# AberHu/TF-NAS

Measured on AMD Instinct MI355X. Metric: supernet search images/sec (w-step + alpha-step), higher is better.
Workload: dtype fp32

## Files before the change

### tf-nas_amd/csrc/gemm_kernels.hip

```cpp
#include <stdlib.h>
#include <string.h>
#include "gemm_core.h"
#include "gemm_x3.h"
#include "kernels.h"
#include "prof.h"

__device__ __forceinline__ f32x4 stem_patch4(const float* __restrict__ img, const TfnasCellDesc& d, int p, int t0) {
    const int HW = d.H * d.W, n = p / HW, r = p - n * HW, ho = r / d.W, wo = r - ho * d.W;
    f32x4 v = zero4();
#pragma unroll
    for (int j = 0; j < 4; ++j) {
        const int t = t0 + j;
        if (t < 27) {
            const int ci = t / 9, rem = t - 9 * ci, ky = rem / 3, kx = rem - 3 * ky;
            const int hi = 2 * ho + ky - 1, wi = 2 * wo + kx - 1;
            if (hi >= 0 && hi < d.Hi && wi >= 0 && wi < d.Wi) v[j] = img[((size_t)(n * 3 + ci) * d.Hi + hi) * d.Wi + wi];
        }
    }
    return v;
}

constexpr int kLbBig = 3, kLbSmall = 4;
constexpr int kLbX3Big = 2, kLbX3Small = 3;
constexpr int gemm_lb(int nt, int mm) { return mm == 0 ? (nt >= 5 ? kLbBig : kLbSmall) : (nt >= 5 ? kLbX3Big : kLbX3Small); }
// ... 460 lines not shown
    const int ocp = (oc + 15) & ~15;
    const int r0 = blockIdx.x * rows_per_split, r1 = min(Po, r0 + rows_per_split);
    const int nchunks = (r1 - r0 + 15) >> 4;
    const int tid = threadIdx.x, lane = tid & 63, lr = lane & 15, lq = lane >> 4, wrow = (tid >> 6) * 32;

    const Bn3Tab tab = bn3_tab_fill(lds + T::LDS_FLOATS, ocp, d, g, stats3, red3, wmix);
    const int mch = m0 + (tid & 31) * 4;
    const bool chok = mch < mcp;
    const size_t acol = (size_t)off + min(mch, mcp - 4);
    float2 c2[4];
#pragma unroll
    for (int j = 0; j < 4; ++j)
        c2[j] = (mch + j < mc) ? bn_consts(stats2 + 2 * (size_t)(off + mch + j), 1.0 / (double)Po, d.eps)
                               : make_float2(0.f, 0.f);
    __syncthreads();
    constexpr int BQ = T::BN / 4;
    int bcol[T::B_ITERS];
    bool bok[T::B_ITERS];
    f32x4 k_mean[T::B_ITERS], k_a3[T::B_ITERS], k_ab[T::B_ITERS], k_s[T::B_ITERS];
#pragma unroll
    for (int i = 0; i < T::B_ITERS; ++i) {
        const int idx = tid + 256 * i, o = n0 + (idx % BQ) * 4;
        bok[i] = idx < T::B_ITEMS && o < oc;
        bcol[i] = min(o, oc - 4);
#pragma unroll
        for (int j = 0; j < 4; ++j) {
            const int oo = bcol[i] + j;
            k_mean[i][j] = tab.mean[oo];
            k_a3[i][j] = tab.a3[oo];
            k_ab[i][j] = tab.a3[oo] * tab.b3[oo];
            k_s[i][j] = tab.rstd[oo] * tab.c3[oo] * tab.a3[oo];
        }
    }
    const float inv_hw = 1.f / (float)HW;
    const bool small_p = Po < (1 << 24);
    auto image_of = [&](int p) -> int {
        if (!small_p) return p / HW;
        int q = (int)((float)p * inv_hw);
        const int r = p - q * HW;
        q += (r >= HW) ? 1 : 0;
        q -= (r < 0) ? 1 : 0;
        return q;
    };

    f32x4 acc[2][NT];
    acc_zero<NT>(acc);
    auto la = [&](int c, int i, int kl, int m) -> Raw2 {
        const int p = min(r0 + c * 16 + kl, r1 - 1);
        Raw2 r;
        r.a = ld4(D + ((size_t)p * M + acol));
        r.b = ld4(gbase + ((size_t)image_of(p) * M + acol) * se01);
        return r;
    };
    auto xa = [&](Raw2 r, int c, int i, int kl, int m) -> f32x4 {
        f32x4 v = r.a;
#pragma unroll
        for (int j = 0; j < 4; ++j) v[j] = act_f<ACT>((v[j] - c2[j].x) * c2[j].y);
        if (has_se) v *= r.b;
        return (chok && r0 + c * 16 + kl < r1) ? v : zero4();
    };
    auto lb = [&](int c, int i, int kl, int n) -> Raw2 {
        const int p = min(r0 + c * 16 + kl, r1 - 1);
        Raw2 r;
        r.a = ld4(dout + (size_t)p * oc + bcol[i]);
        r.b = ld4(Pr + ((size_t)g * Po + p) * oc + bcol[i]);
        return r;
    };
    auto xb = [&](Raw2 r, int c, int i, int kl, int n) -> f32x4 {
        const f32x4 v = (k_a3[i] * r.a - k_ab[i]) - (r.b - k_mean[i]) * k_s[i];
        return (bok[i] && r0 + c * 16 + kl < r1) ? v : zero4();
    };
    gemm_mainloop2<NT, false, false, false>(la, xa, lb, xb, nchunks, acc, lds);
    const bool vec = (mc & 3) == 0;
#pragma unroll
    for (int i = 0; i < 2; ++i) {
        const int ch0 = m0 + wrow + 16 * i + 4 * lq;
#pragma unroll
        for (int j = 0; j < NT; ++j) {
            const int o = n0 + 16 * j + lr;
            if (o >= oc) continue;
            float* dst = gw + (size_t)o * mc + ch0;
            if (vec && ch0 + 3 < mc) {
                st4(dst, acc[i][j]);
            } else {
#pragma unroll
                for (int r = 0; r < 4; ++r)
                    if (ch0 + r < mc) dst[r] = acc[i][j][r];
            }
        }
    }
}

__device__ __forceinline__ f32x4 bn1_de(const f32x4* cb, f32x4 deh, f32x4 e) {
    f32x4 r;
#pragma unroll
    for (int j = 0; j < 4; ++j) {
        const f32x4 t = cb[j];
        const float eh = (e[j] - t.x) * t.y;
        r[j] = t.y * (deh[j] - t.z - eh * t.w);
    }
    return r;
}

__device__ __forceinline__ f32x4 sink_add(f32x4 v, float w, f32x4 g) {
    float px = w * g.x, py = w * g.y, pz = w * g.z, pw = w * g.w;
    asm volatile("" : "+v"(px), "+v"(py), "+v"(pz), "+v"(pw));
    f32x4 r;
    r.x = v.x + px; r.y = v.y + py; r.z = v.z + pz; r.w = v.w + pw;
    return r;
}

template <int NT, int MM>
__global__ __launch_bounds__(256, gemm_lb(NT, MM)) void k_expand_dgrad(TfnasCellDesc d, const float* __restrict__ dEh,
                                                      const float* __restrict__ x, const float* __restrict__ cb1,
                                                      const float* __restrict__ gram, const float* __restrict__ dout,
                                                      const float* __restrict__ wmix, float* __restrict__ dx,
                                                      float* __restrict__ dxp, int nsplit,
                                                      const float* __restrict__ add_src,
                                                      const float* __restrict__ add_scale, int xonly_slot = -1) {
    using T = GT<NT>;
    __shared__ __attribute__((aligned(16))) float lds[T::LDS_FLOATS];
    const int n0 = blockIdx.y * T::BN;
    const int P = d.N * d.H * d.W, ic = d.ic, M = d.M;
    const int nrt = (P + 127) >> 7;
    const int tid = threadIdx.x, lr = tid & 15, wrow = (tid >> 6) * 32;
    const int zs = (int)blockIdx.z;
    int mchunks = 0;
    for (int g = 0; g < d.G; ++g) mchunks += (d.g[g].mcp + 15) >> 4;
    const int nchunks_all = mchunks + ((ic + 15) >> 4);
    const bool xonly = xonly_slot >= 0;
    const int per = xonly ? nchunks_all - mchunks : (nchunks_all + nsplit - 1) / nsplit;
    const int cbeg = xonly ? mchunks : zs * per;
    const int nchunks = max(0, min(nchunks_all, cbeg + per) - cbeg);
    float* __restrict__ dst = xonly ? dxp + (size_t)xonly_slot * P * ic : (nsplit > 1 ? dxp + (size_t)blockIdx.z * P * ic : dx);
    const bool plain = nsplit == 1 && !xonly;
    const bool add_res = d.has_res && plain;
    const bool add_sink = add_src != nullptr && plain;
    const float sink_w = add_src ? add_scale[0] : 0.f;
    float sumw = 1.f;
    if (wmix) {
        sumw = 0.f;
        for (int g = 0; g < d.G; ++g) sumw += wmix[g];
    }

    for (int rt = blockIdx.x; rt < nrt; rt += gridDim.x) {
        f32x4 acc[2][NT];
        acc_zero<NT>(acc);
        bool is_x;
        int k0, klim_a, klim_b, ld_a;
        size_t aoff;
        const float* bsrc;
        const float* ssrc;
        auto pre = [&](int c) {
            c += cbeg;
            if (c >= mchunks) {
                is_x = true;
                k0 = (c - mchunks) * 16;
                klim_a = klim_b = ld_a = ic;
                aoff = 0;
                bsrc = gram;
                ssrc = cb1 + 1;
                return;
            }
            int g = 0;
            for (; g < d.G - 1; ++g) {
                const int t = (d.g[g].mcp + 15) >> 4;
                if (c < t) break;
                c -= t;
            }
            is_x = false;
            k0 = c * 16;
            klim_a = d.g[g].mcp;
            klim_b = d.g[g].mc;
            ld_a = M;
            aoff = d.g[g].off;
            bsrc = d.g[g].w_expand;
            ssrc = cb1 + 4 * (size_t)d.g[g].off + 1;
        };
        int prow[2];
#pragma unroll
        for (int i = 0; i < 2; ++i) prow[i] = rt * 128 + wrow + 16 * i + lr;
        auto la = [&](int c, int i, int kl) -> f32x4 {
            const int pc = min(prow[i], P - 1), k = min(k0 + kl, klim_a - 4);
            return ld4((is_x ? x : dEh) + (size_t)pc * ld_a + aoff + k);
        };
        auto xa = [&](f32x4 r, int c, int i, int kl) -> f32x4 {
            return (prow[i] < P && k0 + kl < klim_a) ? r : zero4();
        };
        auto lb = [&](int c, int kl, int n) -> RawWS {
            const int kc = min(k0 + kl, klim_b - 1), col = min(n0 + n, ic - 4);
            RawWS r;
            r.w = ld4(bsrc + (size_t)kc * ic + col);
            r.s = ssrc[is_x ? 0 : 4 * (size_t)kc];
            return r;
        };
        auto xb = [&](RawWS r, int c, int kl, int n) -> f32x4 {
            const f32x4 v = is_x ? -r.w : splat4(r.s) * r.w;
            return (n0 + n < ic && k0 + kl < klim_b) ? v : zero4();
        };
        gemm_adirect<NT, false, MM>(pre, la, xa, lb, xb, nchunks, acc, lds);
        emit_tile_rows<NT>(acc, lds, [&](int lrow, int lc, f32x4 v) {
            const int p = rt * 128 + lrow, c = n0 + lc;
            if (p < P && c < ic) {
                if (plain) v += ld4(gram + (size_t)ic * ic + c);
                if (add_res) v += splat4(sumw) * ld4(dout + (size_t)p * d.oc + c);
                if (add_sink) v = sink_add(v, sink_w, ld4(add_src + (size_t)p * ic + c));
                st4(dst + (size_t)p * ic + c, v);
            }
        });
    }
}

__global__ __launch_bounds__(256) void k_dx_reduce(TfnasCellDesc d, const float* __restrict__ dxp, int nsplit,
                                                   const float* __restrict__ gram, const float* __restrict__ dout,
                                                   const float* __restrict__ wmix, float* __restrict__ dx,
                                                   const float* __restrict__ add_src,
                                                   const float* __restrict__ add_scale) {
    const float sink_w = add_src ? add_scale[0] : 0.f;
    const size_t n4 = (size_t)d.N * d.H * d.W * d.ic / 4;
    const int iq = d.ic / 4;
    const float* __restrict__ bias = gram + (size_t)d.ic * d.ic;
    float sumw = 1.f;
    if (wmix) {
        sumw = 0.f;
        for (int g = 0; g < d.G; ++g) sumw += wmix[g];
    }
    for (size_t i = (size_t)blockIdx.x * 256 + threadIdx.x; i < n4; i += (size_t)gridDim.x * 256) {
        f32x4 v = ld4(bias + 4 * (int)(i % iq));
        if (d.has_res) v += splat4(sumw) * ld4(dout + 4 * i);
        for (int z = 0; z < nsplit; ++z) v += ld4(dxp + (size_t)z * n4 * 4 + 4 * i);
        if (add_src) v = sink_add(v, sink_w, ld4(add_src + 4 * i));
        st4(dx + 4 * i, v);
    }
}

template <int NT>
__global__ __launch_bounds__(256) void k_expand_gram(TfnasCellDesc d, const float* __restrict__ cb1, int chunks_per_split,
                                                     int nsplit, float* __restrict__ part) {
    using T = GT<NT>;
    __shared__ __attribute__((aligned(16))) float lds[T::LDS_FLOATS];
    const int ic = d.ic;
    const int m0 = blockIdx.y * 128, n0 = blockIdx.z * T::BN;
    const int xs = (int)blockIdx.x;
    int mchunks = 0;
    for (int g = 0; g < d.G; ++g) mchunks += (d.g[g].mcp + 15) >> 4;
    const int cbeg = xs * chunks_per_split;
    const int nchunks = max(0, min(mchunks, cbeg + chunks_per_split) - cbeg);
    const f32x4* cb = reinterpret_cast<const f32x4*>(cb1);
    const int tid = threadIdx.x, lane = tid & 63, lr = lane & 15, lq = lane >> 4, wrow = (tid >> 6) * 32;
    float* __restrict__ out = part + (size_t)blockIdx.x * (size_t)(ic + 4) * ic;

    f32x4 acc[2][NT];
    acc_zero<NT>(acc);
    auto locate = [&](int c, int& g, int& k0) {
        c += cbeg;
        g = 0;
        for (; g < d.G - 1; ++g) {
            const int t = (d.g[g].mcp + 15) >> 4;
            if (c < t) break;
            c -= t;
        }
        k0 = c * 16;
    };
    auto fa = [&](int c, int kl, int m) -> f32x4 {
        int g, k0;
        locate(c, g, k0);
        const int k = k0 + kl, r = m0 + m;
        if (k >= d.g[g].mc || r > ic) return zero4();
        const f32x4 t = cb[d.g[g].off + k];
        const float sk = t.y * t.y * t.w;
        if (r == ic) {
            f32x4 v = zero4();
            v.x = sk * t.x - t.y * t.z;
            return v;
        }
        return splat4(sk) * ld4(d.g[g].w_expand + (size_t)k * ic + r);
    };
    auto fb = [&](int c, int kl, int n) -> f32x4 {
        int g, k0;
        locate(c, g, k0);
        const int k = k0 + kl;
        return (k < d.g[g].mc && n0 + n < ic) ? ld4(d.g[g].w_expand + (size_t)k * ic + n0 + n) : zero4();
    };
    gemm_mainloop<NT, false, false>(fa, fb, nchunks, acc, lds);
#pragma unroll
    for (int i = 0; i < 2; ++i)
#pragma unroll
        for (int r = 0; r < 4; ++r) {
            const int row = m0 + wrow + 16 * i + 4 * lq + r;
            if (row <= ic) {
#pragma unroll
                for (int j = 0; j < NT; ++j) {
                    const int cc = n0 + 16 * j + lr;
                    if (cc < ic) out[(size_t)row * ic + cc] = acc[i][j][r];
                }
            }
        }
}

#ifndef GRAM1_MAX_K
#define GRAM1_MAX_K 1536
#endif
constexpr int GRAM1_GB = 8;
template <int GRAM1_NW>
__global__ __launch_bounds__(64 * GRAM1_NW) void k_gram1(TfnasCellDesc d, const float* __restrict__ cb1, float* __restrict__ gram) {
    __shared__ float part[GRAM1_NW][2][16][17];
    const int ic = d.ic;
    const int r0 = blockIdx.y * 16, c0 = blockIdx.x * 32;
    const int tid = threadIdx.x, wave = tid >> 6, lane = tid & 63, li = lane & 15, kq = lane >> 4;
    const f32x4* cb = reinterpret_cast<const f32x4*>(cb1);
    const int r = r0 + li, ca = c0 + li, cb_ = c0 + 16 + li;
    const bool row_w = r < ic, row_b = r == ic, oka = ca < ic, okb = cb_ < ic;
    const int ra = row_w ? r : 0, caa = oka ? ca : 0, cbb = okb ? cb_ : 0;
    f32x4 acc0 = zero4(), acc1 = zero4();
    int base = 0;
    for (int g = 0; g < d.G; ++g) {
        const float* __restrict__ W = d.g[g].w_expand;
        const int mc = d.g[g].mc, off = d.g[g].off;
        const int nstep = (mc + 3) >> 2, nbatch = (nstep + GRAM1_GB - 1) / GRAM1_GB;
        int b = (wave - base % GRAM1_NW + GRAM1_NW) % GRAM1_NW;
        for (; b < nbatch; b += GRAM1_NW) {
            const int s0 = b * GRAM1_GB;
            float a[GRAM1_GB], b0[GRAM1_GB], b1[GRAM1_GB];
            f32x4 t[GRAM1_GB];
#pragma unroll
            for (int u = 0; u < GRAM1_GB; ++u) {
                const int m = 4 * (s0 + u) + kq;
                const int mm = m < mc ? m : mc - 1;
                const float* wr = W + (size_t)mm * ic;
                t[u] = cb[off + mm];
                a[u] = wr[ra];
                b0[u] = wr[caa];
                b1[u] = wr[cbb];
            }
#pragma unroll
            for (int u = 0; u < GRAM1_GB; ++u) {
                const int m = 4 * (s0 + u) + kq;
                const bool okm = m < mc;
                const float sk = t[u].y * t[u].y * t[u].w;
                float av = row_w ? sk * a[u] : (row_b ? sk * t[u].x - t[u].y * t[u].z : 0.f);
                av = okm ? av : 0.f;
                const float bv0 = (okm && oka) ? b0[u] : 0.f, bv1 = (okm && okb) ? b1[u] : 0.f;
                acc0 = __builtin_amdgcn_mfma_f32_16x16x4f32(av, bv0, acc0, 0, 0, 0);
                acc1 = __builtin_amdgcn_mfma_f32_16x16x4f32(av, bv1, acc1, 0, 0, 0);
            }
        }
        base += nbatch;
    }
#pragma unroll
    for (int q = 0; q < 4; ++q) {
        part[wave][0][4 * kq + q][li] = acc0[q];
        part[wave][1][4 * kq + q][li] = acc1[q];
    }
    __syncthreads();
    for (int e = tid; e < 512; e += 64 * GRAM1_NW) {
        const int h = e >> 8, row = (e >> 4) & 15, col = e & 15;
        double v = 0.0;
#pragma unroll
        for (int w = 0; w < GRAM1_NW; ++w) v += (double)part[w][h][row][col];
        const int rr = r0 + row, cc = c0 + 16 * h + col;
        if (rr <= ic && cc < ic) gram[(size_t)rr * ic + cc] = (float)v;
    }
}

template <int NT, bool STEM, bool XG>
__global__ __launch_bounds__(256, wgrad_lb(NT)) void k_expand_wgrad(TfnasCellDesc d, const float* __restrict__ dEh,
                                                      const float* __restrict__ E, const float* __restrict__ cb1,
                                                      const float* __restrict__ x, int rows_per_split,
                                                      float* __restrict__ part, size_t out_size, size_t out_main) {
    using T = GT<NT>;
    __shared__ __attribute__((aligned(16))) float lds[T::LDS_FLOATS];
    const int ic = d.ic;
    int ty = blockIdx.y, g = 0;
    for (; g < d.G - 1; ++g) {
        const int t = (d.g[g].mcp + 127) >> 7;
        if (ty < t) break;
        ty -= t;
    }
    const int mc = d.g[g].mc, mcp = d.g[g].mcp, off = d.g[g].off;
    const bool last = XG && g == d.G - 1;
    size_t poff = 0;
    for (int gg = 0; gg < g; ++gg) poff += (size_t)d.g[gg].mc * ic;
    float* __restrict__ gw = part + (size_t)blockIdx.x * out_size + poff;
    float* __restrict__ gx = part + (size_t)blockIdx.x * out_size + out_main;
    const int m0 = ty * 128, n0 = blockIdx.z * T::BN;
    const int P = d.N * d.H * d.W, M = d.M;
    const int r0 = blockIdx.x * rows_per_split, r1 = min(P, r0 + rows_per_split);
    const int nchunks = (r1 - r0 + 15) >> 4;
    const int tid = threadIdx.x, lane = tid & 63, lr = lane & 15, lq = lane >> 4, wrow = (tid >> 6) * 32;

    const int mch = m0 + (tid & 31) * 4;
    const bool chok = mch < mcp;
    const size_t acol = (size_t)off + min(mch, mcp - 4);
    f32x4 k_mu = zero4(), k_r = zero4(), k_rt1 = zero4(), k_s = zero4();
    if (!XG) {
#pragma unroll
        for (int j = 0; j < 4; ++j) {
            const f32x4 t = (mch + j < mcp) ? reinterpret_cast<const f32x4*>(cb1)[off + mch + j] : zero4();
            k_mu[j] = t.x;
            k_r[j] = t.y;
            k_rt1[j] = t.y * t.z;
            k_s[j] = t.y * t.y * t.w;
        }
    }
    const int ext = mch - mcp;
    const bool ax = last && ext >= 0 && ext < ic, aone = last && ext == ic;
    const float* __restrict__ abase = ax ? x + ext : dEh + acol;
    const size_t apitch = ax ? (size_t)ic : (size_t)M;
    const bool aok = chok || ax;
    constexpr int BQ = T::BN / 4;
    int bcol[T::B_ITERS];
    bool bok[T::B_ITERS];
#pragma unroll
    for (int i = 0; i < T::B_ITERS; ++i) {
        const int idx = tid + 256 * i, cc = n0 + (idx % BQ) * 4;
        bok[i] = idx < T::B_ITEMS && cc < ic;
        bcol[i] = STEM ? cc : min(cc, ic - 4);
    }

    f32x4 acc[2][NT];
    acc_zero<NT>(acc);
    auto la = [&](int c, int i, int kl, int m) -> Raw2 {
        const int p = min(r0 + c * 16 + kl, r1 - 1);
        Raw2 r;
        if (XG) {
            r.a = ld4(abase + (size_t)p * apitch);
            r.b = r.a;
        } else {
            const size_t at = (size_t)p * M + acol;
            r.a = ld4(dEh + at);
            r.b = ld4(E + at);
        }
        return r;
    };
    auto xa = [&](Raw2 r, int c, int i, int kl, int m) -> f32x4 {
        if (XG) {
            f32x4 v = aok ? r.a : zero4();
            if (aone) v.x = 1.f;
            return (r0 + c * 16 + kl < r1) ? v : zero4();
        }
        const f32x4 v = (k_r * r.a - k_rt1) - (r.b - k_mu) * k_s;
        return (chok && r0 + c * 16 + kl < r1) ? v : zero4();
    };
    auto lb = [&](int c, int i, int kl, int n) -> f32x4 {
        if (STEM) {
            const int p = r0 + c * 16 + kl;
            return (p < r1 && bok[i]) ? stem_patch4(x, d, p, bcol[i]) : zero4();
        }
        const int p = min(r0 + c * 16 + kl, r1 - 1);
        return ld4(x + (size_t)p * ic + bcol[i]);
    };
    auto xb = [&](f32x4 r, int c, int i, int kl, int n) -> f32x4 {
        if (STEM) return r;
        return (bok[i] && r0 + c * 16 + kl < r1) ? r : zero4();
    };
    gemm_mainloop2<NT, false, false, false>(la, xa, lb, xb, nchunks, acc, lds);
#pragma unroll
    for (int i = 0; i < 2; ++i)
#pragma unroll
        for (int r = 0; r < 4; ++r) {
            const int ch = m0 + wrow + 16 * i + 4 * lq + r;
            float* __restrict__ row = nullptr;
            if (ch < mc) row = gw + (size_t)ch * ic;
            else if (last && ch >= mcp && ch - mcp <= ic) row = gx + (size_t)(ch - mcp) * ic;
            if (row) {
#pragma unroll
                for (int j = 0; j < NT; ++j) {
                    const int cc = n0 + 16 * j + lr;
                    if (cc < ic) row[cc] = acc[i][j][r];
                }
            }
        }
}

__global__ __launch_bounds__(256) void k_expand_wgrad_fix(TfnasCellDesc d, const float* __restrict__ cb1,
                                                          const double* __restrict__ red, size_t out_main) {
    __shared__ double ps[4][64];
    const int ic = d.ic, lane = threadIdx.x & 63, wv = threadIdx.x >> 6;
    const size_t e = (size_t)blockIdx.x * 64 + lane;
    const bool ok = e < out_main;
    int g = 0;
    size_t poff = 0;
    for (; g < d.G - 1; ++g) {
        const size_t n = (size_t)d.g[g].mc * ic;
        if (e < poff + n) break;
        poff += n;
    }
    const int m = ok ? (int)((e - poff) / ic) : 0, c = ok ? (int)(e - poff - (size_t)m * ic) : 0;
    const double* __restrict__ Gx = red + out_main;
    const float* __restrict__ w = d.g[g].w_expand + (size_t)m * ic;
    double wg0 = 0.0, wg1 = 0.0;
    for (int k = 4 * wv; k < ic; k += 16) {
        const f32x4 wq = ld4(w + k);
        wg0 += (double)wq.x * Gx[(size_t)k * ic + c] + (double)wq.z * Gx[(size_t)(k + 2) * ic + c];
        wg1 += (double)wq.y * Gx[(size_t)(k + 1) * ic + c] + (double)wq.w * Gx[(size_t)(k + 3) * ic + c];
    }
    ps[wv][lane] = wg0 + wg1;
    __syncthreads();
    if (wv == 0 && ok) {
        const double wg = (ps[0][lane] + ps[1][lane]) + (ps[2][lane] + ps[3][lane]);
        const f32x4 t = reinterpret_cast<const f32x4*>(cb1)[d.g[g].off + m];
        const double sx = Gx[(size_t)ic * ic + c], mu = t.x, r = t.y, t1 = t.z, t2 = t.w;
        const float v = (float)(r * (red[e] - t1 * sx - t2 * r * (wg - mu * sx)));
        float* __restrict__ o = d.g[g].g_expand + (e - poff);
        *o = (d.flags & TFNAS_CELL_ACCUM_WGRAD) ? *o + v : v;
    }
}

static const int kNtSmall[] = {1, 2, 3, 4, 5, 7};
static constexpr int kGtLdsFloats[8] = {0, GT<1>::LDS_FLOATS, GT<2>::LDS_FLOATS, GT<3>::LDS_FLOATS, GT<4>::LDS_FLOATS,
                                        GT<5>::LDS_FLOATS, 0, GT<7>::LDS_FLOATS};

#define NT_CASE(n, ...) case n: { constexpr int NT = n; __VA_ARGS__; } break;
#define DISPATCH_NT_GROUPS(nt, ...)   \
    switch (nt) {                     \
        NT_CASE(4, __VA_ARGS__)       \
        NT_CASE(5, __VA_ARGS__)       \
        NT_CASE(7, __VA_ARGS__)       \
        default: return TFNAS_EINVAL; \
    }
#define DISPATCH_NT(nt, ...)                         \
    switch (nt) {                                    \
        NT_CASE(1, __VA_ARGS__)                      \
        NT_CASE(2, __VA_ARGS__)                      \
        NT_CASE(3, __VA_ARGS__)                      \
        default: DISPATCH_NT_GROUPS(nt, __VA_ARGS__) \
    }
#define DISPATCH_MM(mode, ...)                                 \
    switch (mode) {                                            \
        case 0: { constexpr int MM = 0; __VA_ARGS__; } break;  \
        case 1: { constexpr int MM = 1; __VA_ARGS__; } break;  \
        case 3: { constexpr int MM = 3; __VA_ARGS__; } break;  \
        default: { constexpr int MM = 6; __VA_ARGS__; } break; \
    }
#define DISPATCH_ACT(act, ...) ACT_DISPATCH(act, __VA_ARGS__)

static int g_gemm_mode = 6;
int gemm_mode() { return g_gemm_mode & 7; }
int set_gemm_mode(int m) {
    const int base = m & ~TFNAS_GEMM_EVERYWHERE;
    if (base != 0 && base != 1 && base != 3 && base != 6) return TFNAS_EINVAL;
    g_gemm_mode = m;
    return 0;
}
static inline int gemm_word(const TfnasCellDesc& d) { return (d.gemm_mode & TFNAS_GEMM_EXPLICIT) ? d.gemm_mode : g_gemm_mode; }
int gemm_mode_of(const TfnasCellDesc& d) { return gemm_word(d) & 7; }
static int gemm_arith(const TfnasCellDesc& d, bool dgrad) {
    for (int g = 0; g < d.G; ++g)
        if (d.g[g].mc & 3) return 0;
    const int m = gemm_mode_of(d);
    if (!dgrad || m == 0 || (gemm_word(d) & TFNAS_GEMM_EVERYWHERE)) return m;
    if (m == 1) return m;
    return (d.G > 1 && d.Ho * d.Wo <= 196) ? m : 0;
}
static inline int gemm_slots(int nt, int mm) { return 256 * gemm_lb(nt, mm); }

static size_t stats_row_cap(size_t row_floats) {
    const size_t fit = TFNAS_PART_FLOATS / (row_floats ? row_floats : 1);
    return fit < 1024 ? fit : 1024;
}

static int row_blocks(int rows, int other_blocks, size_t cap, int slots, int max_gx = 1024) {
    const int nrt = cdiv(rows, 128);
    const int other = other_blocks > 0 ? other_blocks : 1;
    int lim = nrt;
    if ((size_t)lim > cap) lim = (int)cap;
    if (lim > max_gx) lim = max_gx;
    if (lim < 1) lim = 1;
    long best_cost = -1;
    int best = 1;
    for (int gx = 1; gx <= lim; ++gx) {
        const long cost = (long)cdiv(gx * other, slots) * cdiv(nrt, gx);
        if (best_cost < 0 || cost <= best_cost) {
            best_cost = cost;
            best = gx;
        }
    }
    return best;
}

static int pick_nt_groups(const TfnasCellDesc& d) {
    int min_mcp = 1 << 30;
    for (int g = 0; g < d.G; ++g) min_mcp = d.g[g].mcp < min_mcp ? d.g[g].mcp : min_mcp;
    if (min_mcp >= 200) return 4;
    static const int cands[] = {4, 5, 7};
    int best = 4;
    long best_pad = -1;
    for (int i = 0; i < 3; ++i) {
        long pad = 0;
        for (int g = 0; g < d.G; ++g) pad += (long)cdiv(d.g[g].mcp, 16 * cands[i]) * 16 * cands[i];
        if (best_pad < 0 || pad < best_pad || (pad == best_pad && cands[i] > best)) {
            best_pad = pad;
            best = cands[i];
        }
    }
    return best;
}
static int group_tiles(const TfnasCellDesc& d, int width, int last_extra = 0) {
    int t = 0;
    for (int g = 0; g < d.G; ++g) t += cdiv(d.g[g].mcp + (g == d.G - 1 ? last_extra : 0), width);
    return t;
}
static int max_mcp(const TfnasCellDesc& d) {
    int m = 0;
    for (int g = 0; g < d.G; ++g) m = d.g[g].mcp > m ? d.g[g].mcp : m;
    return m;
}
static size_t mid_floats(const TfnasCellDesc& d, int n) {
    size_t f = 0;
    for (int g = 0; g < d.G; ++g) f += (size_t)d.g[g].mc * n;
    return f;
}
static GemmPlan plan_cols(int n) {
    GemmPlan p{};
    p.nt = pick_nt(n, kNtSmall, 6);
    p.tiles = cdiv(n, 16 * p.nt);
    return p;
}

GemmPlan gemm_plan_expand_fwd(const TfnasCellDesc& d) {
    GemmPlan p{};
    p.var = d.mode == TFNAS_MODE_STEM ? GEMM_STEM : GEMM_PLAIN;
    p.nt = p.var == GEMM_STEM ? (d.g[0].mcp <= 32 ? 2 : 4) : pick_nt_groups(d);
    p.mm = gemm_arith(d, false);
    p.tiles = group_tiles(d, 16 * p.nt);
    p.grid = dim3(row_blocks(d.N * d.H * d.W, p.tiles, stats_row_cap(2 * (size_t)d.M), gemm_slots(p.nt, p.mm)), p.tiles);
    return p;
}

int launch_expand_fwd(const TfnasCellDesc& d, const float* x, float* E, double* stats1, float* part,
                      hipStream_t s) {
    ProfScope _prof(TK_EXPAND_FWD, s);
    const GemmPlan p = gemm_plan_expand_fwd(d);
    DISPATCH_MM(p.mm, {
        if (p.var == GEMM_STEM)
            hipLaunchKernelGGL((p.nt == 2 ? k_expand_fwd<2, true, MM> : k_expand_fwd<4, true, MM>), p.grid, dim3(256), 0, s, d, x, E, part);
        else
            DISPATCH_NT_GROUPS(p.nt, { hipLaunchKernelGGL((k_expand_fwd<NT, false, MM>), p.grid, dim3(256), 0, s, d, x, E, part); })
    })
    _prof.stop();
    return launch_reduce_rows(part, p.grid.x, 2 * d.M, 2 * (size_t)d.M, stats1, nullptr, s);
}

#ifndef TFNAS_WSPLIT_DGRAD
#define TFNAS_WSPLIT_DGRAD 2
#endif
#ifndef TFNAS_WSPLIT_PFWD
#define TFNAS_WSPLIT_PFWD 2
#endif
GemmPlan gemm_plan_project_fwd(const TfnasCellDesc& d) {
    GemmPlan p = plan_cols(d.oc);
    p.mm = gemm_arith(d, false);
    const int mcp_max = max_mcp(d), ncols2 = 2 * d.G * d.oc;
    const int Po = d.N * d.Ho * d.Wo, nrt = cdiv(Po, 128);
    p.shm = (kGtLdsFloats[p.nt] + 2 * ((mcp_max + 15) & ~15)) * sizeof(float);
    int nsplit = 1;
    const int wgs = nrt * p.tiles * d.G, kch = cdiv(mcp_max, 16);
    if (wgs < 512 && kch >= 16 && (d.oc & 3) == 0 && d.oc <= 1024) {
        nsplit = cdiv(1024, wgs);
        if (nsplit > 4) nsplit = 4;
        if (nsplit > kch / 8) nsplit = kch / 8;
        if (d.need_wgrad && d.G == 1 && nsplit > TFNAS_WSPLIT_PFWD) nsplit = TFNAS_WSPLIT_PFWD;
        const size_t per = (size_t)d.G * Po * d.oc, rows2 = 256 * (size_t)ncols2;
        while (nsplit > 1 && (nsplit - 1) * per + rows2 > TFNAS_PART_FLOATS) --nsplit;
    }
    p.splits = nsplit;
    p.parts = nsplit - 1;
    if (p.parts) p.grid = dim3(nrt, p.tiles, d.G * nsplit);
    else p.grid = dim3(row_blocks(Po, p.tiles * d.G, stats_row_cap((size_t)ncols2), gemm_slots(p.nt, p.mm)), p.tiles, d.G);
    int gx2 = cdiv(Po, 64);
    if (gx2 > 256) gx2 = 256;
    p.rps = cdiv(Po, gx2);
    p.grid2 = dim3(cdiv(Po, p.rps), d.G);
    return p;
}

int launch_project_fwd(const TfnasCellDesc& d, const float* D, const float* gate, const double* stats2,
                       float* Pr, double* stats3, float* part, hipStream_t s) {
    ProfScope _prof(TK_PROJECT_FWD, s);
    const GemmPlan p = gemm_plan_project_fwd(d);
    const int ncols2 = 2 * d.G * d.oc, Po = d.N * d.Ho * d.Wo;
    float* prp = p.parts ? part : nullptr;
    float* rows = part + (size_t)p.parts * d.G * Po * d.oc;
    DISPATCH_MM(p.mm, DISPATCH_NT(p.nt, DISPATCH_ACT(d.act, {
        hipLaunchKernelGGL((k_project_fwd<NT, ACT, MM>), p.grid, dim3(256), p.shm, s, d, D, gate, stats2, Pr, part, p.splits, prp);
    })))
    if (p.parts) hipLaunchKernelGGL(k_pr_reduce, p.grid2, dim3(256), 0, s, Pr, prp, p.parts, d.G, Po, d.oc, p.rps, rows);
    _prof.stop();
    return launch_reduce_rows(rows, p.parts ? p.grid2.x : p.grid.x, ncols2, (size_t)ncols2, stats3, nullptr, s);
}

GemmPlan gemm_plan_project_dgrad(const TfnasCellDesc& d, bool fold) {
    GemmPlan p{};
    p.var = fold ? GEMM_FOLD : GEMM_PLAIN;
    p.nt = pick_nt_groups(d);
    p.mm = gemm_arith(d, true);
    p.tiles = group_tiles(d, 16 * p.nt);
    p.grid = dim3(row_blocks(d.N * d.Ho * d.Wo, p.tiles, 1u << 30, gemm_slots(p.nt, p.mm)), p.tiles);
    p.shm = (kGtLdsFloats[p.nt] + 4 * ((d.oc + 15) & ~15)) * sizeof(float);
    return p;
}

int launch_project_dgrad(const TfnasCellDesc& d, const float* dout, const float* Pr, const double* stats3,
                         const double* red3, const float* wmix, float* dZ, hipStream_t s, const float* D,
                         const double* stats2, float* rec) {
    ProfScope _prof(TK_PROJECT_DGRAD, s);
    if (rec && (!D || !stats2)) return TFNAS_ENULL;
    if (rec && d.act != TFNAS_ACT_RELU && d.act != TFNAS_ACT_SWISH) return TFNAS_EINVAL;
    const GemmPlan p = gemm_plan_project_dgrad(d, rec != nullptr);
    DISPATCH_MM(p.mm, DISPATCH_NT_GROUPS(p.nt, {
        if (p.var == GEMM_FOLD)
            hipLaunchKernelGGL((k_project_dgrad<NT, MM, true>), p.grid, dim3(256), p.shm, s, d, dout, Pr, stats3, red3, wmix, dZ,
                               D, stats2, rec);
        else
            hipLaunchKernelGGL((k_project_dgrad<NT, MM>), p.grid, dim3(256), p.shm, s, d, dout, Pr, stats3, red3, wmix, dZ);
    }))
    return (int)hipGetLastError();
}

static void plan_row_splits(GemmPlan& p, int rows, int mtiles, int ztiles, size_t scratch) {
    const int target = 256 * wgrad_lb(p.nt), min_rows = 128, out_tiles = mtiles * ztiles;
    int splits = target / (out_tiles > 0 ? out_tiles : 1);
    const size_t cap = scratch / (p.out > 0 ? p.out : 1);
    if ((size_t)splits > cap) splits = (int)cap;
    if (splits < 1) splits = 1;
    int rps = cdiv(rows, splits);
    if (rps < min_rows) rps = min_rows;
    p.rps = ((rps + 15) / 16) * 16;
    p.splits = cdiv(rows, p.rps);
    p.grid = dim3(p.splits, mtiles, ztiles);
}
static int reduce_group_wgrads(const TfnasCellDesc& d, const GemmPlan& p, const float* part, int n, float* TfnasGroup::*dst,
                               hipStream_t s) {
    size_t poff = 0;
    for (int g = 0; g < d.G; ++g) {
        const int cols = d.g[g].mc * n;
        int rc = launch_reduce_rows(part + poff, p.splits, cols, p.out, nullptr, d.g[g].*dst, s, wgrad_accum(d));
        if (rc) return rc;
        poff += cols;
    }
    return (int)hipGetLastError();
}

GemmPlan gemm_plan_project_wgrad(const TfnasCellDesc& d) {
    GemmPlan p = plan_cols(d.oc);
    p.out = mid_floats(d, d.oc);
    plan_row_splits(p, d.N * d.Ho * d.Wo, cdiv(max_mcp(d), 128), p.tiles * d.G, TFNAS_PART_FLOATS);
    p.shm = (kGtLdsFloats[p.nt] + 5 * ((d.oc + 15) & ~15)) * sizeof(float);
    return p;
}

int launch_project_wgrad(const TfnasCellDesc& d, const float* dout, const float* Pr, const float* D,
                         const float* gate, const double* stats2, const double* stats3, const double* red3,
                         const float* wmix, float* part, hipStream_t s) {
    ProfScope _prof(TK_PROJECT_WGRAD, s);
    const GemmPlan p = gemm_plan_project_wgrad(d);
    DISPATCH_NT(p.nt, DISPATCH_ACT(d.act, {
        hipLaunchKernelGGL((k_project_wgrad<NT, ACT>), p.grid, dim3(256), p.shm, s, d, dout, Pr, D, gate, stats2,
                           stats3, red3, wmix, p.rps, p.tiles, part, p.out);
    }))
    _prof.stop();
    return reduce_group_wgrads(d, p, part, d.oc, &TfnasGroup::g_proj, s);
}

size_t expand_gram_floats(const TfnasCellDesc& d) { return (size_t)(d.ic + 4) * d.ic; }
static int mid_chunks(const TfnasCellDesc& d) { return group_tiles(d, 16); }

GemmPlan gemm_plan_expand_gram(const TfnasCellDesc& d, size_t scratch_floats) {
    GemmPlan p{};
    if (!(d.route & TFNAS_ROUTE_GRAM2) && mid_floats(d, 1) <= GRAM1_MAX_K) {
        p.var = GEMM_GRAM1;
        p.grid = dim3(cdiv(d.ic, 32), cdiv(d.ic + 1, 16));
        return p;
    }
    p = plan_cols(d.ic);
    const size_t gsz = expand_gram_floats(d);
    const int mchunks = mid_chunks(d), mtiles = cdiv(d.ic + 1, 128);
    int splits = cdiv(512, mtiles * p.tiles);
    if (splits > mchunks / 4) splits = mchunks / 4;
    if ((size_t)splits > scratch_floats / gsz) splits = (int)(scratch_floats / gsz);
    if (splits < 1) splits = 1;
    p.rps = cdiv(mchunks, splits);
    p.splits = cdiv(mchunks, p.rps);
    p.grid = dim3(p.splits, mtiles, p.tiles);
    return p;
}

int launch_expand_gram(const TfnasCellDesc& d, const float* cb1, float* scratch, size_t scratch_floats, float* gram,
                       hipStream_t s) {
    ProfScope _prof(TK_SMALL, s);
    const GemmPlan p = gemm_plan_expand_gram(d, scratch_floats);
    if (p.var == GEMM_GRAM1) {
        for (int g = 0; g < d.G; ++g)
            if (d.g[g].mc < 1) return TFNAS_EINVAL;
        if (d.mode == TFNAS_MODE_HEAD) hipLaunchKernelGGL(k_gram1<16>, p.grid, dim3(1024), 0, s, d, cb1, gram);
        else hipLaunchKernelGGL(k_gram1<4>, p.grid, dim3(256), 0, s, d, cb1, gram);
        return (int)hipGetLastError();
    }
    const size_t gsz = expand_gram_floats(d);
    if (scratch_floats < gsz) return TFNAS_ERANGE;
    DISPATCH_NT(p.nt, { hipLaunchKernelGGL(k_expand_gram<NT>, p.grid, dim3(256), 0, s, d, cb1, p.rps, p.splits, scratch); })
    _prof.stop();
    return launch_reduce_rows(scratch, p.splits, (int)gsz, gsz, nullptr, gram, s);
}

GemmPlan gemm_plan_expand_dgrad(const TfnasCellDesc& d, bool split, int nsl) {
    GemmPlan p = plan_cols(d.ic);
    p.mm = gemm_arith(d, true);
    const int P = d.N * d.H * d.W, out_tiles = cdiv(P, 128) * p.tiles;
    p.splits = 1;
    if (split && nsl < 0 && out_tiles < 512) {
        const int mchunks = mid_chunks(d);
        int ns = cdiv(1024, out_tiles);
        if (ns > 16) ns = 16;
        if (ns > mchunks / 4) ns = mchunks / 4;
        if (d.need_wgrad && d.G == 1 && ns > TFNAS_WSPLIT_DGRAD) ns = TFNAS_WSPLIT_DGRAD;
        p.splits = ns < 1 ? 1 : ns;
    }
    p.grid = dim3(row_blocks(P, p.tiles * p.splits, 1u << 30, gemm_slots(p.nt, p.mm), 4096), p.tiles, p.splits);
    p.parts = nsl >= 0 ? nsl + 1 : (p.splits > 1 ? p.splits : 0);
    size_t blocks = cdiv64((size_t)P * d.ic / 4, 256 * 2);
    p.grid2 = dim3((unsigned)(blocks > 2048 ? 2048 : blocks));
    return p;
}

int launch_expand_dgrad(const TfnasCellDesc& d, const float* dEh, const float* x, const float* cb1, const float* gram,
                        const float* dout, const float* wmix, float* dx, float* dxp, hipStream_t s,
                        const float* add_src, const float* add_scale, int nsl) {
    const GemmPlan p = gemm_plan_expand_dgrad(d, dxp != nullptr, nsl);
    {
        ProfScope _prof(TK_EXPAND_DGRAD, s);
        DISPATCH_MM(p.mm, DISPATCH_NT(p.nt, {
            hipLaunchKernelGGL((k_expand_dgrad<NT, MM>), p.grid, dim3(256), 0, s, d, dEh, x, cb1, gram, dout, wmix, dx, dxp, p.splits,
                               add_src, add_scale, nsl);
        }))
    }
    if (p.parts) {
        ProfScope _p2(TK_SMALL, s);
        hipLaunchKernelGGL(k_dx_reduce, p.grid2, dim3(256), 0, s, d, dxp, p.parts, gram, dout, wmix, dx, add_src, add_scale);
    }
    return (int)hipGetLastError();
}

static size_t xg_red_floats(const GemmPlan& p) { return p.var == GEMM_XG ? 2 * p.out + 4 : 0; }

GemmPlan gemm_plan_expand_wgrad(const TfnasCellDesc& d) {
    GemmPlan p = plan_cols(d.ic);
    const int P = d.N * d.H * d.W;
    if (d.mode == TFNAS_MODE_STEM) p.var = GEMM_STEM;
    else if (!(d.route & TFNAS_ROUTE_XG_OFF) && (d.ic & 3) == 0 &&
             ((d.route & TFNAS_ROUTE_XG_ALL) || (size_t)P * d.M * sizeof(float) >= ((size_t)100 << 20)))
        p.var = GEMM_XG;
    const int next = p.var == GEMM_XG ? d.ic + 1 : 0;
    p.out_main = mid_floats(d, d.ic);
    p.out = p.out_main + (size_t)next * d.ic;
    plan_row_splits(p, P, group_tiles(d, 128, next), p.tiles, TFNAS_PART_FLOATS - xg_red_floats(p));
    return p;
}

int launch_expand_wgrad(const TfnasCellDesc& d, const float* dEh, const float* E, const float* cb1,
                        const float* x, float* part, hipStream_t s) {
    ProfScope _prof(TK_EXPAND_WGRAD, s);
    const GemmPlan p = gemm_plan_expand_wgrad(d);
    const size_t red_floats = xg_red_floats(p);
    if (p.var != GEMM_XG && !E) return TFNAS_ENULL;
    if (red_floats + p.out > TFNAS_PART_FLOATS) return TFNAS_ERANGE;
    if (p.var == GEMM_STEM && p.nt != 2) return TFNAS_EINVAL;
    DISPATCH_NT(p.nt, {
        auto k = p.var == GEMM_XG ? k_expand_wgrad<NT, false, true> : k_expand_wgrad<NT, false, false>;
        if (p.var == GEMM_STEM) k = k_expand_wgrad<2, true, false>;
        hipLaunchKernelGGL(k, p.grid, dim3(256), 0, s, d, dEh, E, cb1, x, p.rps, part, p.out, p.out_main);
    })
    _prof.stop();
    if (p.var != GEMM_XG) return reduce_group_wgrads(d, p, part, d.ic, &TfnasGroup::g_expand, s);
    double* red = reinterpret_cast<double*>((uintptr_t)(part + TFNAS_PART_FLOATS - red_floats + 3) & ~(uintptr_t)15);
    int rc = launch_reduce_rows(part, p.splits, (int)p.out, p.out, red, nullptr, s);
    if (rc) return rc;
    ProfScope _p2(TK_EXPAND_WGRAD, s);
    hipLaunchKernelGGL(k_expand_wgrad_fix, dim3((unsigned)cdiv64(p.out_main, 64)), dim3(256), 0, s, d, cb1, red, p.out_main);
    return (int)hipGetLastError();
}
```

Before: 3969.

## Parameterize gram1 column tile width and flatten group/batch wave scheduling

The gram1 kernel gets a template column-tile count NT. Non-head cells now use 16-column tiles instead of 32, which doubles the grid along x for more parallelism. Head mode keeps 32 columns. The nested per-group loop with modular wave offsets is replaced by a flat batch index walked across groups, balancing waves over the global batch list. The wave index is made uniform with readfirstlane. A few products are pinned in registers to control codegen, at the cost of more A-operand reloads across column tiles.

```diff
diff --git a/tf-nas_amd/csrc/gemm_kernels.hip b/tf-nas_amd/csrc/gemm_kernels.hip
--- a/tf-nas_amd/csrc/gemm_kernels.hip
+++ b/tf-nas_amd/csrc/gemm_kernels.hip
@@ -786,64 +786,77 @@
 #define GRAM1_MAX_K 1536
 #endif
 constexpr int GRAM1_GB = 8;
-template <int GRAM1_NW>
+template <int GRAM1_NW, int NT>
 __global__ __launch_bounds__(64 * GRAM1_NW) void k_gram1(TfnasCellDesc d, const float* __restrict__ cb1, float* __restrict__ gram) {
-    __shared__ float part[GRAM1_NW][2][16][17];
-    const int ic = d.ic;
-    const int r0 = blockIdx.y * 16, c0 = blockIdx.x * 32;
-    const int tid = threadIdx.x, wave = tid >> 6, lane = tid & 63, li = lane & 15, kq = lane >> 4;
+    __shared__ float part[GRAM1_NW][NT][16][17];
+    const int ic = d.ic, G = d.G;
+    const int r0 = blockIdx.y * 16, c0 = blockIdx.x * 16 * NT;
+    const int tid = threadIdx.x, lane = tid & 63, li = lane & 15, kq = lane >> 4;
+    const int wave = __builtin_amdgcn_readfirstlane(tid >> 6);
     const f32x4* cb = reinterpret_cast<const f32x4*>(cb1);
-    const int r = r0 + li, ca = c0 + li, cb_ = c0 + 16 + li;
-    const bool row_w = r < ic, row_b = r == ic, oka = ca < ic, okb = cb_ < ic;
-    const int ra = row_w ? r : 0, caa = oka ? ca : 0, cbb = okb ? cb_ : 0;
-    f32x4 acc0 = zero4(), acc1 = zero4();
-    int base = 0;
-    for (int g = 0; g < d.G; ++g) {
+    const int r = r0 + li;
+    const bool row_w = r < ic, row_b = r == ic;
+    const int ra = row_w ? r : 0;
+    bool okc[NT];
+    int cc[NT];
+    f32x4 acc[NT];
+#pragma unroll
+    for (int j = 0; j < NT; ++j) {
+        const int c = c0 + 16 * j + li;
+        okc[j] = c < ic;
+        cc[j] = okc[j] ? c : 0;
+        acc[j] = zero4();
+    }
+    int g = 0, b = wave;
+    for (;; b += GRAM1_NW) {
+        int mc = 0;
+        for (; g < G; ++g) {
+            mc = d.g[g].mc;
+            const int nbatch = (((mc + 3) >> 2) + GRAM1_GB - 1) / GRAM1_GB;
+            if (b < nbatch) break;
+            b -= nbatch;
+        }
+        if (g == G) break;
         const float* __restrict__ W = d.g[g].w_expand;
-        const int mc = d.g[g].mc, off = d.g[g].off;
-        const int nstep = (mc + 3) >> 2, nbatch = (nstep + GRAM1_GB - 1) / GRAM1_GB;
-        int b = (wave - base % GRAM1_NW + GRAM1_NW) % GRAM1_NW;
-        for (; b < nbatch; b += GRAM1_NW) {
-            const int s0 = b * GRAM1_GB;
-            float a[GRAM1_GB], b0[GRAM1_GB], b1[GRAM1_GB];
-            f32x4 t[GRAM1_GB];
-#pragma unroll
-            for (int u = 0; u < GRAM1_GB; ++u) {
-                const int m = 4 * (s0 + u) + kq;
-                const int mm = m < mc ? m : mc - 1;
-                const float* wr = W + (size_t)mm * ic;
-                t[u] = cb[off + mm];
-                a[u] = wr[ra];
-                b0[u] = wr[caa];
-                b1[u] = wr[cbb];
-            }
-#pragma unroll
-            for (int u = 0; u < GRAM1_GB; ++u) {
-                const int m = 4 * (s0 + u) + kq;
-                const bool okm = m < mc;
-                const float sk = t[u].y * t[u].y * t[u].w;
-                float av = row_w ? sk * a[u] : (row_b ? sk * t[u].x - t[u].y * t[u].z : 0.f);
-                av = okm ? av : 0.f;
-                const float bv0 = (okm && oka) ? b0[u] : 0.f, bv1 = (okm && okb) ? b1[u] : 0.f;
-                acc0 = __builtin_amdgcn_mfma_f32_16x16x4f32(av, bv0, acc0, 0, 0, 0);
-                acc1 = __builtin_amdgcn_mfma_f32_16x16x4f32(av, bv1, acc1, 0, 0, 0);
-            }
-        }
-        base += nbatch;
-    }
-#pragma unroll
-    for (int q = 0; q < 4; ++q) {
-        part[wave][0][4 * kq + q][li] = acc0[q];
-        part[wave][1][4 * kq + q][li] = acc1[q];
-    }
+        const int off = d.g[g].off, s0 = b * GRAM1_GB;
+        float a[GRAM1_GB], bw[NT][GRAM1_GB];
+        f32x4 t[GRAM1_GB];
+#pragma unroll
+        for (int u = 0; u < GRAM1_GB; ++u) {
+            const int m = 4 * (s0 + u) + kq;
+            const int mm = m < mc ? m : mc - 1;
+            const float* wr = W + (size_t)mm * ic;
+            t[u] = cb[off + mm];
+            a[u] = wr[ra];
+#pragma unroll
+            for (int j = 0; j < NT; ++j) bw[j][u] = wr[cc[j]];
+        }
+#pragma unroll
+        for (int u = 0; u < GRAM1_GB; ++u) {
+            const int m = 4 * (s0 + u) + kq;
+            const bool okm = m < mc;
+            const float sk = t[u].y * t[u].y * t[u].w;
+            float bx = sk * t[u].x, byz = t[u].y * t[u].z;
+            asm("" : "+v"(bx), "+v"(byz));
+            float av = row_w ? sk * a[u] : (row_b ? bx - byz : 0.f);
+            av = okm ? av : 0.f;
+#pragma unroll
+            for (int j = 0; j < NT; ++j)
+                acc[j] = __builtin_amdgcn_mfma_f32_16x16x4f32(av, (okm && okc[j]) ? bw[j][u] : 0.f, acc[j], 0, 0, 0);
+        }
+    }
+#pragma unroll
+    for (int j = 0; j < NT; ++j)
+#pragma unroll
+        for (int q = 0; q < 4; ++q) part[wave][j][4 * kq + q][li] = acc[j][q];
     __syncthreads();
-    for (int e = tid; e < 512; e += 64 * GRAM1_NW) {
+    for (int e = tid; e < 256 * NT; e += 64 * GRAM1_NW) {
         const int h = e >> 8, row = (e >> 4) & 15, col = e & 15;
         double v = 0.0;
 #pragma unroll
         for (int w = 0; w < GRAM1_NW; ++w) v += (double)part[w][h][row][col];
-        const int rr = r0 + row, cc = c0 + 16 * h + col;
-        if (rr <= ic && cc < ic) gram[(size_t)rr * ic + cc] = (float)v;
+        const int rr = r0 + row, cn = c0 + 16 * h + col;
+        if (rr <= ic && cn < ic) gram[(size_t)rr * ic + cn] = (float)v;
     }
 }
 
@@ -1254,7 +1267,8 @@
     GemmPlan p{};
     if (!(d.route & TFNAS_ROUTE_GRAM2) && mid_floats(d, 1) <= GRAM1_MAX_K) {
         p.var = GEMM_GRAM1;
-        p.grid = dim3(cdiv(d.ic, 32), cdiv(d.ic + 1, 16));
+        p.nt = d.mode == TFNAS_MODE_HEAD ? 2 : 1;
+        p.grid = dim3(cdiv(d.ic, 16 * p.nt), cdiv(d.ic + 1, 16));
         return p;
     }
     p = plan_cols(d.ic);
@@ -1277,8 +1291,8 @@
     if (p.var == GEMM_GRAM1) {
         for (int g = 0; g < d.G; ++g)
             if (d.g[g].mc < 1) return TFNAS_EINVAL;
-        if (d.mode == TFNAS_MODE_HEAD) hipLaunchKernelGGL(k_gram1<16>, p.grid, dim3(1024), 0, s, d, cb1, gram);
-        else hipLaunchKernelGGL(k_gram1<4>, p.grid, dim3(256), 0, s, d, cb1, gram);
+        if (p.nt == 2) hipLaunchKernelGGL((k_gram1<16, 2>), p.grid, dim3(1024), 0, s, d, cb1, gram);
+        else hipLaunchKernelGGL((k_gram1<4, 1>), p.grid, dim3(256), 0, s, d, cb1, gram);
         return (int)hipGetLastError();
     }
     const size_t gsz = expand_gram_floats(d);
```

After: 3968. Within noise of the previous version (-0.0%).
